# vbarbosadev/MatrixFactorizationSGD.java

Hardware: AMD Instinct MI355X
Metric: rating-updates/sec (higher is better)
Workload: dtype f32; 1 GPU; cfg2_ml20m (MovieLens-20M shape, Zipf-Mandelbrot degrees); workload_rev=2, users_per_gpu=138493, items=26744, nnz_per_gpu=20000000, nnz_global=20000000, users_global=138493, k=64, max_item_degree=67853, sum_round_steps=51381, blocks=256, waves=2, parts_per_rank=1, emulated_world=0, parallelism=single

## Files before the change

### matrixfactorizationsgd.java_amd/csrc/cell.hpp

```cpp
#pragma once

#include <hip/hip_runtime.h>

#include <cstdint>

#include "canon.hpp"
#include "records.hpp"
#include "run_asm.hpp"

#pragma clang fp contract(off)

namespace mfsgd {
namespace {

__device__ __forceinline__ void wg_barrier() { asm volatile("s_waitcnt lgkmcnt(0)\n\ts_barrier" ::: "memory"); }

using gptr_t = const __attribute__((address_space(1))) void*;
using lptr_t = __attribute__((address_space(3))) void*;
using f32x4 = __attribute__((ext_vector_type(4))) float;

__device__ __forceinline__ float4 lds_ld(const unsigned char* base, unsigned off) {
    return *reinterpret_cast<const float4*>(base + off);
}
__device__ __forceinline__ void lds_st(unsigned char* base, unsigned off, const float4 v) {
    *reinterpret_cast<float4*>(base + off) = v;
}

template <int EST, int L>
__device__ __forceinline__ void run_loop_asm(float4& rq, const unsigned ea, const unsigned rowbase, int pairs,
                                             const float lr) {
    static_assert(L == 16 || L == 32 || L == 64, "hand-scheduled run loop: 16, 32 or 64 lanes per rating");
    using f4 = __attribute__((ext_vector_type(4))) float;
    f4 q = {rq.x, rq.y, rq.z, rq.w};
    constexpr int PADV = mfsgd_pad_run(L);
    if constexpr (L == 16)
        asm volatile(MFSGD_RUN_LOOP_ASM_TEXT("", MFSGD_SFMA_V) MFSGD_RUN_LOOP_ASM_OPERANDS);
    else if constexpr (L == 32)
        asm volatile(MFSGD_RUN_LOOP_ASM_TEXT(MFSGD_SWAP_ADD16, MFSGD_SFMA_V) MFSGD_RUN_LOOP_ASM_OPERANDS);
    else
        asm volatile(MFSGD_RUN_LOOP_ASM_TEXT(MFSGD_BCAST_ADD64, MFSGD_SFMA_S) MFSGD_RUN_LOOP_ASM_OPERANDS);
    rq = make_float4(q[0], q[1], q[2], q[3]);
}

template <int EST, int L>
__device__ __forceinline__ void gen_loop_asm(const unsigned ea, const unsigned rowbase, int n, const float lr, const uint64_t c2) {
    static_assert(L == 16 || L == 32 || L == 64, "hand-scheduled general loop: 16, 32 or 64 lanes per rating");
    n = __builtin_amdgcn_readfirstlane(n);
    constexpr int PADV = mfsgd_pad_gen(L);
    if constexpr (L == 16)
        asm volatile(MFSGD_GEN_LOOP_ASM_TEXT("", MFSGD_SFMA_V) MFSGD_GEN_LOOP_ASM_OPERANDS);
    else if constexpr (L == 32)
        asm volatile(MFSGD_GEN_LOOP_ASM_TEXT(MFSGD_SWAP_ADD16, MFSGD_SFMA_V) MFSGD_GEN_LOOP_ASM_OPERANDS);
    else
        asm volatile(MFSGD_GEN_LOOP_ASM_TEXT(MFSGD_BCAST_ADD64, MFSGD_SFMA_S) MFSGD_GEN_LOOP_ASM_OPERANDS);
}

template <int L>
__device__ __forceinline__ void solo_chain_asm(float4& rq, const unsigned ea, const unsigned s0, const unsigned rowbase, int n,
                                               const float lr, const uint64_t c2) {
    static_assert(L == 16 || L == 32 || L == 64, "solo loops: 16, 32 or 64 lanes per rating");
    using f4 = __attribute__((ext_vector_type(4))) float;
    f4 q;
    n = __builtin_amdgcn_readfirstlane(n);
    constexpr int PADV = mfsgd_pad_chain_tail(L), PADS = mfsgd_pad_chain_steady(L);
    if constexpr (L == 16)
        asm volatile(MFSGD_SOLO_CHAIN_ASM_TEXT("", MFSGD_SFMA2_V) MFSGD_SOLO_CHAIN_OPERANDS);
    else if constexpr (L == 32)
        asm volatile(MFSGD_SOLO_CHAIN_ASM_TEXT(MFSGD_BCAST_ADD32, MFSGD_SFMA2_S) MFSGD_SOLO_CHAIN_OPERANDS);
    else
        asm volatile(MFSGD_SOLO_CHAIN_ASM_TEXT(MFSGD_BCAST_ADD64, MFSGD_SFMA2_S) MFSGD_SOLO_CHAIN_OPERANDS);
    rq = make_float4(q[0], q[1], q[2], q[3]);
}
template <int L>
__device__ __forceinline__ bool solo_helper_asm(const unsigned ea, const unsigned rowbase, int n, const uint64_t c2,
                                                int fin = 1) {
    constexpr int PADV = mfsgd_pad_helper(L);
    n = __builtin_amdgcn_readfirstlane(n);
    fin = __builtin_amdgcn_readfirstlane(fin);
    asm volatile("" : "+s"(fin));
    int spins = 1 << 22;
    asm volatile(MFSGD_SOLO_HELPER_ASM_TEXT MFSGD_SOLO_HELPER_OPERANDS);
    return spins != 0;
}

template <int L, int W>
constexpr int epoch_helpers() {
    return W <= 4 ? W : 0;
}

__device__ __forceinline__ CellDesc load_desc(const CellDesc* __restrict__ cells, unsigned idx) {
    idx = (unsigned)__builtin_amdgcn_readfirstlane((int)idx);
    asm volatile("" : "+s"(idx));
    return cells[idx];
}

template <int L, int W, int NH = 0>
struct Cell {
    static constexpr int G = 64 / L;
    static constexpr int ROWB = 16 * L;
    static constexpr int KP = 4 * L;
    static constexpr int NWV = W + NH;
    static constexpr int NT = 64 * NWV;
    static constexpr int CTL = 16;
    static constexpr int SUBB = (W * W * 8 + 15) & ~15;

    int tid, lane, wave, g, lig;
    int wave_all;
    bool helper;
    unsigned laneoff;
    int nu, nrows, n_steps;
    bool critical;
    volatile unsigned* fail_flag = nullptr;
    unsigned long long* post_at = nullptr;
    unsigned post_tag = 0;
    volatile unsigned* posted_flag = nullptr;
    unsigned char* lrows;
    uint4* lent;
    uint2* lsub;
    uint32_t* lids;

    __device__ __forceinline__ void init_thread() {
        tid = threadIdx.x;
        lane = tid & 63;
        wave_all = __builtin_amdgcn_readfirstlane(tid >> 6);
        helper = NH > 0 && wave_all >= W;
        wave = helper ? wave_all - W : wave_all;
        g = lane / L;
        lig = lane % L;
        laneoff = (unsigned)lig * 16u;
    }
    __device__ __forceinline__ void bind(const CellDesc& cd, unsigned char* smem, int buf, int sched_cap) {
        nu = cd.nu;
        nrows = (int)cd.nu + (int)cd.ni;
        n_steps = (int)(cd.n_steps & 0x7FFFFFFFu);
        critical = (cd.n_steps >> 31) != 0;
        lrows = smem + CTL + 2 * (size_t)sched_cap;
        lent = reinterpret_cast<uint4*>(smem + CTL + (size_t)buf * sched_cap);
        lsub = reinterpret_cast<uint2*>(lent + (size_t)n_steps * G);
        lids = reinterpret_cast<uint32_t*>(reinterpret_cast<unsigned char*>(lsub) + SUBB);
    }

    __device__ __forceinline__ void zero_idle_rows() {
        for (int x = tid; x < 2 * G * L; x += NT)
            lds_st(lrows, (unsigned)(nrows * ROWB + x * 16), make_float4(0.f, 0.f, 0.f, 0.f));
    }

    __device__ __forceinline__ void prefetch_schedule(const CellDesc& nd, int ncell, unsigned char* smem, int buf,
                                                      int sched_cap, const uint32_t* __restrict__ rows,
                                                      const SubDesc* __restrict__ subs,
                                                      const Entry* __restrict__ entries) {
        unsigned char* const dst = smem + CTL + (size_t)buf * sched_cap;
        const int nn = (int)nd.nu + (int)nd.ni;
        const int ent_bytes = (int)(nd.n_steps & 0x7FFFFFFFu) * G * 16;
        const int sub_bytes = SUBB;
        const int ids_bytes = (nn * 4 + 15) & ~15;
        auto copy = [&](const unsigned char* src, unsigned char* d, int bytes) {
            for (int off0 = wave_all * 1024; off0 < bytes; off0 += NWV * 1024) {
                const int off = off0 + lane * 16;
                if (off < bytes)
                    __builtin_amdgcn_global_load_lds((gptr_t)(src + off), (lptr_t)(d + off0), 16, 0, 0);
            }
        };
        copy(reinterpret_cast<const unsigned char*>(entries + (size_t)nd.ent_off * G), dst, ent_bytes);
        copy(reinterpret_cast<const unsigned char*>(subs + (size_t)ncell * W * W), dst + ent_bytes, sub_bytes);
        copy(reinterpret_cast<const unsigned char*>(rows + nd.row_off), dst + ent_bytes + sub_bytes, ids_bytes);
    }

    __device__ __forceinline__ void stage_schedule(const CellDesc& cd, int cell, const uint32_t* __restrict__ rows,
                                                   const SubDesc* __restrict__ subs,
                                                   const Entry* __restrict__ entries) {
        const uint32_t* const crow = rows + cd.row_off;
        for (int x = tid; x < nrows; x += NT) lids[x] = crow[x];
        const uint4* gent = reinterpret_cast<const uint4*>(entries) + (size_t)cd.ent_off * G;
        const int ne = n_steps * G;
        for (int x = tid; x < ne; x += NT) lent[x] = gent[x];
        if (tid < W * W) lsub[tid] = reinterpret_cast<const uint2*>(subs)[(size_t)cell * W * W + tid];
        zero_idle_rows();
    }

    template <bool COH = false>
    __device__ __forceinline__ void gather(const float* __restrict__ P, const float* __restrict__ Q, int lo, int hi) {
        constexpr int AUX = COH ? 16 : 0;
        constexpr int UNR = 4;
        const int first = (lo / G) * G;
        int s0 = first + wave_all * G;
        for (; s0 + (UNR - 1) * NWV * G < hi; s0 += UNR * NWV * G) {
            uint32_t rid[UNR];
            bool in[UNR];
#pragma unroll
            for (int x = 0; x < UNR; ++x) {
                const int sx = s0 + x * NWV * G + g;
                in[x] = sx >= lo && sx < hi;
                rid[x] = lids[in[x] ? sx : lo];
            }
#pragma unroll
            for (int x = 0; x < UNR; ++x) {
                const int sb = s0 + x * NWV * G;
                if (in[x]) {
                    const float* src = (sb + g < nu ? P : Q) + (size_t)rid[x] * KP + lig * 4;
                    __builtin_amdgcn_global_load_lds((gptr_t)src, (lptr_t)(lrows + (size_t)sb * ROWB), 16, 0, AUX);
                }
            }
        }
        for (; s0 < hi; s0 += NWV * G) {
            const int sx = s0 + g;
            if (sx >= lo && sx < hi) {
                const uint32_t rid = lids[sx];
                const float* src = (sx < nu ? P : Q) + (size_t)rid * KP + lig * 4;
                __builtin_amdgcn_global_load_lds((gptr_t)src, (lptr_t)(lrows + (size_t)s0 * ROWB), 16, 0, AUX);
            }
        }
    }

    template <bool WT>
    __device__ __forceinline__ void scatter(float* __restrict__ P, float* __restrict__ Q, int lo, int hi) {
        constexpr int UNR = 4;
        auto put = [&](int s, uint32_t rid, const float4 v) {
            float* dst = (s < nu ? P : Q) + (size_t)rid * KP + lig * 4;
            if constexpr (WT) {
                const f32x4 vv = {v.x, v.y, v.z, v.w};
                asm volatile("s_nop 1\n\tglobal_store_dwordx4 %0, %1, off sc1\n\ts_nop 1" ::"v"(dst), "v"(vv) : "memory");
            } else {
                *reinterpret_cast<float4*>(dst) = v;
            }
        };
        int s = lo + wave_all * G + g;
        for (; s + (UNR - 1) * NWV * G < hi; s += UNR * NWV * G) {
            uint32_t rid[UNR];
            float4 v[UNR];
#pragma unroll
            for (int x = 0; x < UNR; ++x) {
                rid[x] = lids[s + x * NWV * G];
                v[x] = lds_ld(lrows, (unsigned)((s + x * NWV * G) * ROWB) + laneoff);
            }
#pragma unroll
            for (int x = 0; x < UNR; ++x) put(s + x * NWV * G, rid[x], v[x]);
        }
        for (; s < hi; s += NWV * G) put(s, lids[s], lds_ld(lrows, (unsigned)(s * ROWB) + laneoff));
    }

    struct Sub {
        int n, nr;
        int offs;
        __device__ __forceinline__ int first() const { return offs & 0xFFFF; }
        __device__ __forceinline__ int nsolo() const { return (int)((unsigned)offs >> 16); }
    };
    __device__ __forceinline__ Sub sub(const int x) const {
        const uint2 sd = lsub[x];
        const int nall = __builtin_amdgcn_readfirstlane((int)sd.y);
        return Sub{nall & 0xFFFF, (int)((unsigned)nall >> 16), __builtin_amdgcn_readfirstlane((int)sd.x)};
    }
    static __device__ __forceinline__ uint64_t pack_c2(const float c) {
        return ((uint64_t)__builtin_bit_cast(unsigned, c) << 32) | __builtin_bit_cast(unsigned, c);
    }
    static __device__ __forceinline__ unsigned row_base(unsigned char* rows, const unsigned lo) {
        return (unsigned)(uintptr_t)(lptr_t)rows + lo;
    }
    static constexpr bool kAsmLoops = L == 16 || L == 32 || L == 64;

    struct StepRegs {
        uint4 en;
        unsigned pa, qa;
        float4 p, q;
    };

    template <bool TRAIN, bool TIMED = false>
    __device__ __forceinline__ void apply(const float lr, const float c, double& acc,
                                          unsigned long long* timers = nullptr) {
        unsigned char* const lr_ = lrows;
        const unsigned lo = laneoff;
        if constexpr (NH > 0 && TRAIN) {
            if (helper) {
                for (int s = 0; s < W; ++s) {
                    if constexpr (L >= 16) {
                        auto run_of = [&](const int a, int& ns) -> const uint4* {
                            const uint2 sd = lsub[s * W + a];
                            ns = __builtin_amdgcn_readfirstlane((int)(sd.x >> 16));
                            const int first = __builtin_amdgcn_readfirstlane((int)((sd.x & 0xFFFFu) + (sd.y & 0xFFFFu) + (sd.y >> 16))) + kSoloPad;
                            return lent + (size_t)first * G;
                        };
                        int ns;
                        const uint4* hdr = run_of((wave + 1) % W, ns);
                        if (ns > 0 && !solo_helper_asm<L>((unsigned)(uintptr_t)(lptr_t)hdr, row_base(lr_, lo), ns, pack_c2(c)) && fail_flag)
                            *fail_flag = 1;
                    }
                    wg_barrier();
                }
                return;
            }
        }
        auto set_addr = [&](StepRegs& x) {
            x.pa = ((x.en.x & 0xFFFFu) << 4) + lo;
            x.qa = (__builtin_amdgcn_ubfe(x.en.x, 16, 15) << 4) + lo;
        };
        auto step = [&](StepRegs& cur, StepRegs& nxt, const uint4* eptr, const int e2) {
            __builtin_amdgcn_sched_barrier(0);
            asm volatile("" : "+v"(nxt.en.x));
            const float r = __builtin_bit_cast(float, TRAIN ? cur.en.z : cur.en.y);
            set_addr(nxt);
            const float4 pn = lds_ld(lr_, nxt.pa);
            const float4 qn = lds_ld(lr_, nxt.qa);
            cur.en = eptr[e2];
            __builtin_amdgcn_sched_barrier(0);
            const float dot = group_allreduce<L>(chunk_dot(cur.p, cur.q));
            if constexpr (TRAIN) {
                const float sc = __builtin_fmaf(-lr, dot, r);
                const float4 p2 = axpy_row(sc, cur.q, c, cur.p);
                const float4 q2 = axpy_row(sc, cur.p, c, cur.q);
                lds_st(lr_, cur.pa, p2);
                lds_st(lr_, cur.qa, q2);
                const bool fwd = (int)nxt.en.x < 0;
                nxt.q.x = fwd ? q2.x : qn.x;
                nxt.q.y = fwd ? q2.y : qn.y;
                nxt.q.z = fwd ? q2.z : qn.z;
                nxt.q.w = fwd ? q2.w : qn.w;
            } else {
                const float err = r - dot;
                acc += (double)err * (double)err;
                nxt.q = qn;
            }
            nxt.p = pn;
// ... 145 lines not shown
```

### matrixfactorizationsgd.java_amd/csrc/epoch.hip

```cpp
#include <hip/hip_runtime.h>

#include <cstdint>

#include "cell.hpp"
#include "dispatch.hpp"
#include "kernels.hpp"

#pragma clang fp contract(off)

namespace mfsgd {

namespace {

constexpr int kFlagStride = 32;

using gu32 = __attribute__((address_space(1))) unsigned;
using gu64 = __attribute__((address_space(1))) unsigned long long;

__device__ __forceinline__ unsigned start_barrier(unsigned* __restrict__ done, unsigned* __restrict__ abort_word,
                                                  const int B, const int wg, const int NP, unsigned& my_gen) {
    unsigned bad = __hip_atomic_load((gu32*)abort_word, __ATOMIC_RELAXED, __HIP_MEMORY_SCOPE_AGENT);
    my_gen = 0;
    if (bad == 0u) {
        gu32* arrive = (gu32*)(abort_word - 4);
// ... 65 lines not shown
__device__ __forceinline__ void post_row(gu64* dst, const unsigned long long tag, const int lane,
                                         const unsigned char* row) {
#pragma unroll
    for (int j = 0; j < NGR; ++j) {
        const unsigned bits = *reinterpret_cast<const unsigned*>(row + (size_t)(lane + 64 * j) * 4);
        __hip_atomic_store(dst + 64 * j, tag | bits, __ATOMIC_RELAXED, __HIP_MEMORY_SCOPE_AGENT);
    }
}

template <int L, int W, int NH>
__device__ __forceinline__ void run_ring(unsigned char* smem, float* __restrict__ P, float* __restrict__ Q,
                                         const CellDesc* __restrict__ cells, const uint32_t* __restrict__ rows,
                                         const SubDesc* __restrict__ subs, const Entry* __restrict__ entries,
                                         const int B, const int n_rounds, const float lr, const float c,
                                         unsigned* __restrict__ done, unsigned* __restrict__ abort_word,
                                         const int sched_cap, const int wg, const int NP,
                                         unsigned long long* __restrict__ prof) {
    volatile unsigned* const ctl = reinterpret_cast<volatile unsigned*>(smem);
    Cell<L, W, NH> cx;
    cx.init_thread();
    cx.fail_flag = ctl;
    cx.posted_flag = ctl + 3;
    if (cx.tid == 0) {
        unsigned my_gen;
        const unsigned bad = start_barrier(done, abort_word, B, wg, NP, my_gen);
        ctl[0] = bad != 0u ? 1u : 0u;
        ctl[1] = bad;
        ctl[2] = my_gen;
    }
    wg_barrier();
    if (ctl[0] != 0) return;
    gu64* const mbox = (gu64*)(abort_word + 4);
    const unsigned tag_hi = ctl[2] << 16;
    constexpr int KP = Cell<L, W, NH>::KP, ROWB = Cell<L, W, NH>::ROWB;
    constexpr int NGR = KP >= 64 ? KP / 64 : 1;

    struct Item {
        int R, b;
        unsigned idx;
        bool first;
    };
    auto cell_of = [&](int R, int b) { return (unsigned)(b * B + (b + R % B) % B); };
    auto next_item = [&](const Item& it, const CellDesc& d) {
        Item n = it;
        if (d.next != 0) {
            n.idx = d.next;
            n.first = false;
        } else {
            n.b += NP;
            if (n.b >= B) {
                n.b = wg;
                ++n.R;
            }
            n.idx = cell_of(n.R, n.b);
            n.first = true;
        }
        return n;
    };
    Item it0{0, wg, cell_of(0, wg), true};
    CellDesc cd = load_desc(cells, it0.idx);
    Item it1 = next_item(it0, cd);
    CellDesc cd1 = it1.R < n_rounds ? load_desc(cells, it1.idx) : cd;
    int buf = 0;
    cx.bind(cd, smem, buf, sched_cap);
    cx.stage_schedule(cd, (int)it0.idx, rows, subs, entries);
    asm volatile("s_waitcnt vmcnt(0)" ::: "memory");
    wg_barrier();

    unsigned long long pacc[8] = {0, 0, 0, 0, 0, 0, 0, 0};
    unsigned long long pcur[7] = {0, 0, 0, 0, 0, 0, 0}, pmax[7] = {0, 0, 0, 0, 0, 0, 0};
    unsigned long long pt = 0;
    auto mark = [&](int k) {
        if (prof) {
            const unsigned long long now = __builtin_amdgcn_s_memtime();
            pacc[k] += now - pt;
            pcur[k] = now - pt;
            if (k == 6 && pcur[4] > pacc[7]) {
                pacc[7] = pcur[4];
                for (int x = 0; x < 7; ++x) pmax[x] = pcur[x];
            }
            pt = now;
        }
    };
    if (prof) pt = __builtin_amdgcn_s_memtime();

    for (; it0.R < n_rounds;) {
        const int R = it0.R, b = it0.b;
        CellDesc cd2 = cd1;
        cx.bind(cd, smem, buf, sched_cap);
        const bool work = cx.nrows != 0;
        const bool last = cd.next == 0;
        cx.zero_idle_rows();
        if (cx.tid == 0) ctl[3] = 0u;
        asm volatile("s_waitcnt vmcnt(0)" ::: "memory");
#ifdef MFSGD_DIAG_SPLIT_PHASE0
        mark(0);
#endif
        if (it1.R < n_rounds) cx.prefetch_schedule(cd1, (int)it1.idx, smem, buf ^ 1, sched_cap, rows, subs, entries);
        if (work) cx.gather(P, Q, 0, cx.nu);
        const Item it2 = next_item(it1, cd1);
        const bool lone = KP >= 64 && (cd.rsv[0] & kCellLoneTile) != 0;
#ifdef MFSGD_DIAG_SPLIT_PHASE0
        mark(2);
#endif
        if (it2.R < n_rounds) cd2 = load_desc(cells, it2.idx);
#ifdef MFSGD_DIAG_SPLIT_PHASE0
        mark(6);
#else
        mark(0);
#endif
        if (R > 0 && it0.first && lone) {
            if (cx.wave_all == 0) {
                const unsigned tile = (unsigned)((b + R % B) % B);
                const unsigned want = tag_hi | (unsigned)R;
                const gu64* src = mbox + (size_t)tile * KP + cx.lane;
                unsigned long long v[NGR];
                unsigned spins = 0;
                for (;;) {
                    bool ok = true;
#pragma unroll
                    for (int j = 0; j < NGR; ++j) {
                        v[j] = __hip_atomic_load(src + 64 * j, __ATOMIC_RELAXED, __HIP_MEMORY_SCOPE_AGENT);
                        ok = ok && (unsigned)(v[j] >> 32) == want;
                    }
                    if (__builtin_amdgcn_ballot_w64(!ok) == 0ull) break;
                    __builtin_amdgcn_s_sleep(1);
                    if ((++spins & 255u) == 0u) {
                        if (__hip_atomic_load((gu32*)abort_word, __ATOMIC_RELAXED, __HIP_MEMORY_SCOPE_AGENT) != 0u ||
                            spins > (1u << 22)) {
                            if (cx.lane == 0) {
                                __hip_atomic_store((gu32*)abort_word, 1u, __ATOMIC_RELAXED, __HIP_MEMORY_SCOPE_AGENT);
                                ctl[0] = 1;
                            }
                            break;
                        }
                    }
                }
#pragma unroll
                for (int j = 0; j < NGR; ++j)
                    *reinterpret_cast<unsigned*>(cx.lrows + (size_t)cx.nu * ROWB + (size_t)(cx.lane + 64 * j) * 4) = (unsigned)v[j];
            }
        } else if (R > 0 && it0.first) {
            if (cx.tid == 0) {
                wait_flag((gu32*)(done + (size_t)((b + 1) % B) * kFlagStride), (unsigned)R, abort_word, ctl);
            }
        }
        mark(1);
        const bool from_mbox = lone && R > 0;
        wg_barrier();
        mark(2);
        if (ctl[0] != 0) {
            if (cx.tid == 0) __hip_atomic_store((gu32*)abort_word, 1u, __ATOMIC_RELAXED, __HIP_MEMORY_SCOPE_AGENT);
            return;
        }
        if (work && !from_mbox) cx.template gather<true>(P, Q, cx.nu, cx.nrows);
        if (work) {
            asm volatile("s_waitcnt vmcnt(0)" ::: "memory");
            wg_barrier();
            mark(3);
            double acc = 0.0;
            if (lone && R + 1 < n_rounds) {
                cx.post_at = (unsigned long long*)(abort_word + 4) + (size_t)((b + R % B) % B) * KP;
                cx.post_tag = tag_hi | (unsigned)(R + 1);
            } else {
                cx.post_at = nullptr;
            }
            cx.template apply<true>(lr, c, acc);
            mark(4);
            if (lone && R + 1 < n_rounds) {
                if (cx.wave_all == 0 && ctl[3] == 0u) {
                    const unsigned tile = (unsigned)((b + R % B) % B);
                    const unsigned long long tag = (unsigned long long)(tag_hi | (unsigned)(R + 1)) << 32;
                    post_row<NGR>(mbox + (size_t)tile * KP + cx.lane, tag, cx.lane, cx.lrows + (size_t)cx.nu * ROWB);
                }
            } else {
                cx.template scatter<true>(P, Q, cx.nu, cx.nrows);
            }
        }
        asm volatile("s_waitcnt vmcnt(0)" ::: "memory");
        wg_barrier();
        if (last && cx.tid == 0)
            __hip_atomic_store((gu32*)(done + (size_t)b * kFlagStride), (unsigned)(R + 1), __ATOMIC_RELAXED,
                               __HIP_MEMORY_SCOPE_AGENT);
        mark(5);
        if (work) cx.template scatter<false>(P, Q, 0, cx.nu);
        wg_barrier();
        buf ^= 1;
        cd = cd1;
        cd1 = cd2;
        it0 = it1;
        it1 = it2;
        mark(6);
    }
    if (ctl[0] != 0 && cx.tid == 0)
        __hip_atomic_store((gu32*)abort_word, 1u, __ATOMIC_RELAXED, __HIP_MEMORY_SCOPE_AGENT);
    if (wg == 0 && cx.tid == 0)
        __hip_atomic_fetch_add((gu32*)(abort_word + 1), 1u, __ATOMIC_RELAXED, __HIP_MEMORY_SCOPE_AGENT);
    if (prof && cx.tid == 0) {
        for (int k = 0; k < 8; ++k) prof[(size_t)wg * 16 + k] = pacc[k];
        for (int k = 0; k < 7; ++k) prof[(size_t)wg * 16 + 8 + k] = pmax[k];
    }
}

template <int L, int W>
__global__ void __launch_bounds__(64 * (W + epoch_helpers<L, W>()))
epoch_kernel(float* __restrict__ P, float* __restrict__ Q, const CellDesc* __restrict__ cells,
             const uint32_t* __restrict__ rows, const SubDesc* __restrict__ subs,
             const Entry* __restrict__ entries, const int B, const int n_rounds, const float lr,
             const float c, unsigned* __restrict__ done, unsigned* __restrict__ abort_word,
             const int sched_cap, unsigned long long* __restrict__ prof) {
    extern __shared__ __attribute__((aligned(16))) unsigned char smem[];
    run_ring<L, W, epoch_helpers<L, W>()>(smem, P, Q, cells, rows, subs, entries, B, n_rounds, lr, c, done, abort_word,
                                           sched_cap, (int)blockIdx.x, (int)gridDim.x, prof);
}

template <int L, int W>
hipError_t epoch_grant_lds(const CellLaunch& a) {
    return hipFuncSetAttribute((const void*)epoch_kernel<L, W>, hipFuncAttributeMaxDynamicSharedMemorySize, a.lds_bytes);
}

template <int L, int W>
hipError_t epoch_occupancy_LW(const CellLaunch& a, int* blocks_per_cu) {
    const hipError_t e = epoch_grant_lds<L, W>(a);
    if (e != hipSuccess) return e;
    return hipOccupancyMaxActiveBlocksPerMultiprocessor(blocks_per_cu, (const void*)epoch_kernel<L, W>,
                                                        64 * (W + epoch_helpers<L, W>()), (size_t)a.lds_bytes);
}

template <int L, int W>
hipError_t epoch_launch_LW(const CellLaunch& a, int n_rounds, unsigned* done, unsigned* abort_word, hipStream_t st) {
    const hipError_t e = epoch_grant_lds<L, W>(a);
    if (e != hipSuccess) return e;
    hipLaunchKernelGGL((epoch_kernel<L, W>), dim3((unsigned)a.grid), dim3(64 * (W + epoch_helpers<L, W>())),
                       (size_t)a.lds_bytes, st, a.P, a.Q, a.cells, a.rows, a.subs, a.entries, a.B, n_rounds, a.lr, a.c, done,
                       abort_word, a.sched_cap, reinterpret_cast<unsigned long long*>(a.diag ? a.sse_partial : nullptr));
    return hipGetLastError();
}

}

hipError_t epoch_blocks_per_cu(int L, int W, const CellLaunch& a, int* blocks_per_cu) {
    return with_L(L, [&](auto l) { return with_W(W, [&](auto w) { return epoch_occupancy_LW<l(), w()>(a, blocks_per_cu); }); });
}

hipError_t launch_epoch_persistent(int L, int W, const CellLaunch& a, int n_rounds, unsigned* done,
                                   unsigned* abort_word, hipStream_t st) {
    return with_L(L, [&](auto l) {
        return with_W(W, [&](auto w) { return epoch_launch_LW<l(), w()>(a, n_rounds, done, abort_word, st); });
    });
}

}
```

### matrixfactorizationsgd.java_amd/csrc/run_asm.hpp

```cpp
#pragma once

constexpr int mfsgd_pad_run(int lanes) {
#ifdef MFSGD_PAD_RUN
    return MFSGD_PAD_RUN;
#else
    return 2;
#endif
}
constexpr int mfsgd_pad_gen(int lanes) {
#ifdef MFSGD_PAD_GEN
    return MFSGD_PAD_GEN;
#else
    return 0;
#endif
}
constexpr int mfsgd_pad_chain_steady(int lanes) {
#ifdef MFSGD_PAD_CHAIN_STEADY
    return MFSGD_PAD_CHAIN_STEADY;
#else
    return 0;
#endif
}
constexpr int mfsgd_pad_chain_tail(int lanes) {
#ifdef MFSGD_PAD_CHAIN_TAIL
// ... 144 lines not shown
        EXTRA \
        SFMA(LRR) \
        "v_pk_fma_f32 v[" NQ0 ":" NQ1 "], v[130:131], v[" P0 ":" P1 "], v[122:123] op_sel_hi:[0,1,1]\n\t" \
        "v_pk_fma_f32 v[" NQ2 ":" NQ3 "], v[130:131], v[" P2 ":" P3 "], v[124:125] op_sel_hi:[0,1,1]\n\t" \
        "v_pk_fma_f32 v[134:135], v[130:131], v[" Q0 ":" Q1 "], v[126:127] op_sel_hi:[0,1,1]\n\t" \
        "v_pk_fma_f32 v[136:137], v[130:131], v[" Q2 ":" Q3 "], v[128:129] op_sel_hi:[0,1,1]\n\t" \
        "s_sub_u32 %[n], %[n], 1\n\t" \
        "v_cmp_gt_i32 vcc, 0, v" SLOT_NEXT "\n\t" \
        "ds_write_b128 v" PADDR ", v[134:137]\n\t" \
        "ds_write_b128 v" QADDR ", v[" NQ0 ":" NQ3 "]\n\t" \
        "s_cmp_eq_u32 %[n], 0\n\t" \
        "s_waitcnt lgkmcnt(4)\n\t" \
        "v_cndmask_b32 v" NQ0 ", v144, v" NQ0 ", vcc\n\t" \
        "v_cndmask_b32 v" NQ1 ", v145, v" NQ1 ", vcc\n\t" \
        "v_cndmask_b32 v" NQ2 ", v146, v" NQ2 ", vcc\n\t" \
        "v_cndmask_b32 v" NQ3 ", v147, v" NQ3 ", vcc\n\t"

#define MFSGD_GEN_LOOP_ASM_TEXT(EXTRA, SFMA) \
        "v_mov_b32 v138, %[ea]\n\t" \
        "v_mov_b32 v131, %[lr]\n\t" \
        "v_mov_b32 v139, %[rb]\n\t" \
        "ds_read_b32 v114, v138\n\t" \
        "ds_read_b32 v116, v138 offset:8\n\t" \
        "ds_read_b32 v115, v138 offset:%c[e1]\n\t" \
        "s_waitcnt lgkmcnt(2)\n\t" \
        "v_mad_u32_u16 v112, v114, 16, v139\n\t" \
        "v_bfe_u32 v133, v114, 16, 15\n\t" \
        "v_lshl_add_u32 v148, v133, 4, v139\n\t" \
        "ds_read_b128 v[104:107], v112\n\t" \
        "ds_read_b128 v[100:103], v148\n\t" \
        "ds_write_b32 v138, v114\n\t" \
        "ds_write_b32 v138, v114\n\t" \
        MFSGD_LOOP_ALIGN \
        "1:\n\t" \
        MFSGD_GEN_HALF("104", "105", "106", "107", "100", "101", "102", "103", "112", "148", "108", "111", "140", "141", "142", "143", \
                       "113", "149", "115", "114", "%c[e2]", "116", "117", "%c[e1p8]", EXTRA, SFMA) \
        "s_cbranch_scc1 2f\n\t" \
        MFSGD_GEN_HALF("108", "109", "110", "111", "140", "141", "142", "143", "113", "149", "104", "107", "100", "101", "102", "103", \
                       "112", "148", "114", "115", "%c[e3]", "117", "116", "%c[e2p8]", EXTRA, SFMA) \
        "v_add_u32 v138, %c[e2], v138\n\t" \
        "s_cbranch_scc0 1b\n\t" \
        "2:\n\t" \
        "s_waitcnt lgkmcnt(0)\n\t"

#define MFSGD_GEN_LOOP_ASM_OPERANDS                                                                                    \
    : [n] "+s"(n)                                                                                                      \
    : [ea] "v"(ea), [rb] "v"(rowbase), [lr] "s"(lr), [c2] "s"(c2), [e1] "n"(EST), [e2] "n"(2 * EST), [e3] "n"(3 * EST), \
      [e1p8] "n"(EST + 8), [e2p8] "n"(2 * EST + 8), [pad] "n"(PADV)                                                    \
    : "memory", "scc", "vcc", "v100", "v101", "v102", "v103", "v104", "v105", "v106", "v107", "v108", "v109", "v110", "v111", \
      "v112", "v113", "v114", "v115", "v116", "v117", "v120", "v121", "v122", "v123", "v124", "v125", "v126", "v127",  \
      "v128", "v129", "v130", "v131", "v132", "v133", "v134", "v135", "v136", "v137", "v138", "v139", "v140", "v141",  \
      "v142", "v143", "v144", "v145", "v146", "v147", "v148", "v149"

#define MFSGD_SOLO_CHAIN_HALF(P0, P1, P2, P3, N0, N1, N2, N3, ELRR, ESLOT, NEXTE, OFF_NEXT, WAIT, S, S1, GAP, EXTRA, SFMA) \
        "s_waitcnt lgkmcnt(" WAIT ")\n\t" \
        "v_pk_mul_f32 v[120:121], v[" P0 ":" P1 "], v[100:101]\n\t" \
        "v_pk_fma_f32 v[120:121], v[" P2 ":" P3 "], v[102:103], v[120:121]\n\t" \
        "v_add_f32 v132, v120, v121\n\t" \
        "v_mad_u32_u16 v113, v" ESLOT ", 16, v139\n\t" \
        "v_pk_mul_f32 v[122:123], v[100:101], %[c2]\n\t" \
        "v_add_f32_dpp v132, v132, v132 quad_perm:[1,0,3,2] row_mask:0xf bank_mask:0xf bound_ctrl:1\n\t" \
        "ds_read_b128 v[" N0 ":" N3 "], v113\n\t" \
        "v_pk_mul_f32 v[124:125], v[102:103], %[c2]\n\t" \
        "v_add_f32_dpp v132, v132, v132 quad_perm:[2,3,0,1] row_mask:0xf bank_mask:0xf bound_ctrl:1\n\t" \
        "ds_read2_b32 v[" NEXTE "], v138 " OFF_NEXT "\n\t" \
        "s_nop 0\n\t" \
        "v_add_f32_dpp v132, v132, v132 row_half_mirror row_mask:0xf bank_mask:0xf bound_ctrl:1\n\t" \
        GAP \
        "v_add_f32_dpp v132, v132, v132 row_mirror row_mask:0xf bank_mask:0xf bound_ctrl:1\n\t" \
        EXTRA \
        SFMA(S, ELRR) \
        "v_pk_fma_f32 v[100:101], v[" S ":" S1 "], v[" P0 ":" P1 "], v[122:123] op_sel_hi:[0,1,1]\n\t" \
        "v_pk_fma_f32 v[102:103], v[" S ":" S1 "], v[" P2 ":" P3 "], v[124:125] op_sel_hi:[0,1,1]\n\t"

#define MFSGD_SOLO_CHAIN_GAP_COUNT "s_sub_u32 %[n], %[n], 1\n\ts_cmp_eq_u32 %[n], 0\n\t"
#define MFSGD_SOLO_CHAIN_GAP_NOP "s_nop 1\n\t"
#define MFSGD_SOLO_CHAIN_GAP_PASS \
        ".if 2 * \\j + 2 < %c[steady]\n\ts_nop 1\n\t.else\n\ts_sub_u32 %[n], %[n], %c[steady]\n\ts_cmp_ge_u32 %[n], %c[steady]\n\t.endif\n\t"
#define MFSGD_SOLO_CHAIN_PAIR(GAP_A, GAP_B, EXIT_A, EXTRA, SFMA) \
        MFSGD_SOLO_CHAIN_HALF("104", "105", "106", "107", "108", "109", "110", "111", "116", "117", "118:119", "offset0:6+8*\\j offset1:4+8*\\j", "1", "130", "131", GAP_A, EXTRA, SFMA) \
        EXIT_A \
        MFSGD_SOLO_CHAIN_HALF("108", "109", "110", "111", "104", "105", "106", "107", "118", "119", "116:117", "offset0:10+8*\\j offset1:8+8*\\j", "0", "128", "129", GAP_B, EXTRA, SFMA) \
        "ds_write2_b32 v138, v130, v128 offset0:1+8*\\j offset1:5+8*\\j\n\t"
#define MFSGD_SOLO_CHAIN_ASM_TEXT(EXTRA, SFMA) \
        "v_mov_b32 v138, %[ea]\n\t" \
        "v_mov_b32 v131, %[lr]\n\t" \
        "v_mov_b32 v139, %[rb]\n\t" \
        "ds_read2_b32 v[116:117], v138 offset0:6 offset1:4\n\t" \
        "v_mad_u32_u16 v113, %[s0], 16, v139\n\t" \
        "v_bfe_u32 v133, %[s0], 16, 15\n\t" \
        "ds_read_b128 v[104:107], v113\n\t" \
        "v_lshl_add_u32 v133, v133, 4, v139\n\t" \
        "ds_read_b128 v[100:103], v133\n\t" \
        "ds_write_b32 v138, %[s0]\n\t" \
        "v_add_u32 v138, 16, v138\n\t" \
        "s_cmp_lt_u32 %[n], %c[steady]\n\t" \
        "s_cbranch_scc1 1f\n\t" \
        MFSGD_LOOP_ALIGN_STEADY \
        "5:\n\t" \
        ".irp j,0,1,2,3,4,5,6,7\n\t" \
        ".if 2 * \\j < %c[steady]\n\t" \
        MFSGD_SOLO_CHAIN_PAIR(MFSGD_SOLO_CHAIN_GAP_NOP, MFSGD_SOLO_CHAIN_GAP_PASS, "", EXTRA, SFMA) \
        ".endif\n\t" \
        ".endr\n\t" \
        "v_add_u32 v138, %c[sbump], v138\n\t" \
        "s_cbranch_scc1 5b\n\t" \
        "s_cmp_eq_u32 %[n], 0\n\t" \
        "s_cbranch_scc1 3f\n\t" \
        "s_branch 1f\n\t" \
        MFSGD_LOOP_ALIGN \
        "1:\n\t" \
        ".irp j,0,1,2,3\n\t" \
        ".if \\j < %c[pairs]\n\t" \
        MFSGD_SOLO_CHAIN_PAIR(MFSGD_SOLO_CHAIN_GAP_COUNT, MFSGD_SOLO_CHAIN_GAP_COUNT, "s_cbranch_scc1 2\\j\\()f\n\t", EXTRA, SFMA) \
        ".if \\j + 1 < %c[pairs]\n\t" \
        "s_cbranch_scc1 3f\n\t" \
        ".endif\n\t" \
        ".endif\n\t" \
        ".endr\n\t" \
        "v_add_u32 v138, %c[bump], v138\n\t" \
        "s_cbranch_scc0 1b\n\t" \
        "s_branch 3f\n\t" \
        ".irp j,3,2,1,0\n\t" \
        ".if \\j < %c[pairs]\n\t" \
        "2\\j:\n\t" \
        "ds_write_b32 v138, v130 offset:4+32*\\j\n\t" \
        ".if \\j > 0\n\t" \
        "s_branch 3f\n\t" \
        ".endif\n\t" \
        ".endif\n\t" \
        ".endr\n\t" \
        "3:\n\t" \
        "s_waitcnt lgkmcnt(0)\n\t" \
        "v_mov_b32 %[q0], v100\n\t" \
        "v_mov_b32 %[q1], v101\n\t" \
        "v_mov_b32 %[q2], v102\n\t" \
        "v_mov_b32 %[q3], v103\n\t"

#define MFSGD_SOLO_CHAIN_OPERANDS                                                                                      \
    : [n] "+s"(n), [q0] "=v"(q[0]), [q1] "=v"(q[1]), [q2] "=v"(q[2]), [q3] "=v"(q[3])                                  \
    : [ea] "v"(ea), [rb] "v"(rowbase), [s0] "v"(s0), [lr] "s"(lr), [c2] "s"(c2), [pad] "n"(PADV),                      \
      [pads] "n"(PADS), [pairs] "n"(mfsgd_chain_pairs()), [bump] "n"(32 * mfsgd_chain_pairs()),                         \
      [steady] "n"(mfsgd_chain_steady()), [sbump] "n"(16 * mfsgd_chain_steady())                                       \
    : "memory", "scc", "vcc", "v100", "v101", "v102", "v103", "v104", "v105", "v106", "v107", "v108", "v109", "v110", "v111", \
      "v113", "v116", "v117", "v118", "v119", "v120", "v121", "v122", "v123", "v124", "v125", "v128", "v129", "v130",  \
      "v131", "v132", "v133", "v138", "v139"

#define MFSGD_SOLO_HELPER_PAIR(TAG, M0, M1, M2, M3, N0, N3) \
        "s_waitcnt lgkmcnt(1)\n\t" \
        "v_max_u32 v133, v" M1 ", v" M3 "\n\t" \
        "v_mad_u32_u16 v113, v" M0 ", 16, v139\n\t" \
        "v_cmp_eq_u32 vcc, -1, v133\n\t" \
        "v_pk_mul_f32 v[126:127], v[104:105], %[c2]\n\t" \
        "s_cbranch_vccnz 7" TAG "f\n\t" \
        "6" TAG ":\n\t" \
        "ds_read_b128 v[108:111], v113\n\t" \
        "v_pk_mul_f32 v[128:129], v[106:107], %[c2]\n\t" \
        "ds_read2_b64 v[" N0 ":" N3 "], v138 offset0:4 offset1:6\n\t" \
        "v_pk_mul_f32 v[122:123], v[100:101], %[c2]\n\t" \
        "v_pk_mul_f32 v[124:125], v[102:103], %[c2]\n\t" \
        "v_pk_fma_f32 v[134:135], v[" M0 ":" M1 "], v[100:101], v[126:127] op_sel:[1,0,0]\n\t" \
        "v_pk_fma_f32 v[136:137], v[" M0 ":" M1 "], v[102:103], v[128:129] op_sel:[1,0,0]\n\t" \
        "v_pk_fma_f32 v[100:101], v[" M0 ":" M1 "], v[104:105], v[122:123] op_sel:[1,0,0]\n\t" \
        "v_pk_fma_f32 v[102:103], v[" M0 ":" M1 "], v[106:107], v[124:125] op_sel:[1,0,0]\n\t" \
        "s_sub_u32 %[n], %[n], 2\n\t" \
        "ds_write_b128 v112, v[134:137]\n\t" \
        "v_mad_u32_u16 v112, v" M2 ", 16, v139\n\t" \
        "s_waitcnt lgkmcnt(2)\n\t" \
        "ds_read_b128 v[104:107], v112\n\t" \
        "v_pk_mul_f32 v[126:127], v[108:109], %[c2]\n\t" \
        "v_pk_mul_f32 v[128:129], v[110:111], %[c2]\n\t" \
        "v_pk_mul_f32 v[122:123], v[100:101], %[c2]\n\t" \
        "v_pk_mul_f32 v[124:125], v[102:103], %[c2]\n\t" \
        "v_pk_fma_f32 v[134:135], v[" M2 ":" M3 "], v[100:101], v[126:127] op_sel:[1,0,0]\n\t" \
        "v_pk_fma_f32 v[136:137], v[" M2 ":" M3 "], v[102:103], v[128:129] op_sel:[1,0,0]\n\t" \
        "v_pk_fma_f32 v[100:101], v[" M2 ":" M3 "], v[108:109], v[122:123] op_sel:[1,0,0]\n\t" \
        "v_pk_fma_f32 v[102:103], v[" M2 ":" M3 "], v[110:111], v[124:125] op_sel:[1,0,0]\n\t" \
        "v_add_u32 v138, 32, v138\n\t" \
        "s_cmp_lt_u32 %[n], 2\n\t" \
        "ds_write_b128 v113, v[134:137]\n\t"

#define MFSGD_SOLO_HELPER_SLOW(TAG, M0, M1, M3) \
        "7" TAG ":\n\t" \
        "s_sleep 1\n\t" \
        "ds_read2_b64 v[" M0 ":" M3 "], v138 offset1:2\n\t" \
        "s_sub_u32 %[spins], %[spins], 1\n\t" \
        "s_cmp_eq_u32 %[spins], 0\n\t" \
        "s_cbranch_scc1 9f\n\t" \
        "s_waitcnt lgkmcnt(0)\n\t" \
        "v_max_u32 v133, v" M1 ", v" M3 "\n\t" \
        "v_cmp_eq_u32 vcc, -1, v133\n\t" \
        "s_cbranch_vccnz 7" TAG "b\n\t" \
        "s_branch 6" TAG "b\n\t"

#define MFSGD_SOLO_HELPER_TAIL(TAG, M0, M1) \
        "8" TAG ":\n\t" \
        "s_cmp_eq_u32 %[n], 0\n\t" \
        "s_cbranch_scc1 40f\n\t" \
        "s_waitcnt lgkmcnt(0)\n\t" \
        "v_pk_mul_f32 v[126:127], v[104:105], %[c2]\n\t" \
        "v_pk_mul_f32 v[128:129], v[106:107], %[c2]\n\t" \
        "v_pk_mul_f32 v[122:123], v[100:101], %[c2]\n\t" \
        "v_pk_mul_f32 v[124:125], v[102:103], %[c2]\n\t" \
        "3" TAG ":\n\t" \
        "v_cmp_eq_u32 vcc, -1, v" M1 "\n\t" \
        "s_cbranch_vccz 2" TAG "f\n\t" \
        "s_sleep 1\n\t" \
        "ds_read_b32 v" M1 ", v138 offset:4\n\t" \
        "s_sub_u32 %[spins], %[spins], 1\n\t" \
        "s_cmp_eq_u32 %[spins], 0\n\t" \
        "s_cbranch_scc1 9f\n\t" \
        "s_waitcnt lgkmcnt(0)\n\t" \
        "s_branch 3" TAG "b\n\t" \
        "2" TAG ":\n\t" \
        "v_pk_fma_f32 v[134:135], v[" M0 ":" M1 "], v[100:101], v[126:127] op_sel:[1,0,0]\n\t" \
        "v_pk_fma_f32 v[136:137], v[" M0 ":" M1 "], v[102:103], v[128:129] op_sel:[1,0,0]\n\t" \
        "v_pk_fma_f32 v[100:101], v[" M0 ":" M1 "], v[104:105], v[122:123] op_sel:[1,0,0]\n\t" \
        "v_pk_fma_f32 v[102:103], v[" M0 ":" M1 "], v[106:107], v[124:125] op_sel:[1,0,0]\n\t" \
        "s_nop 0\n\t" \
        "ds_write_b128 v112, v[134:137]\n\t"

#define MFSGD_SOLO_HELPER_ASM_TEXT \
        "v_mov_b32 v141, %[ea]\n\t" \
        "v_mov_b32 v139, %[rb]\n\t" \
        "ds_read_b32 v133, v141\n\t" \
        "v_add_u32 v138, 16, v141\n\t" \
        "3:\n\t" \
        "ds_read2_b64 v[116:119], v138 offset1:2\n\t" \
        "s_waitcnt lgkmcnt(0)\n\t" \
// ... 42 lines not shown
```

Before: 5.441 billion updates/s.

## Fuse lone-tile mailbox poll, solo chain and row post into one asm loop

Adds a fast path for lone tiles whose round contains only a solo chain. One inline-asm block now polls the mailbox for the incoming row, runs the solo SGD chain on it and posts the updated row to the next tile's mailbox. This removes the separate poll loop, the barriers, the gather/apply dispatch and the post_row pass on the critical inter-block handoff chain. The cost is much more hand-written asm, extra clobbered VGPRs, and narrower eligibility checks that fall back to the old path.

```diff
diff --git a/matrixfactorizationsgd.java_amd/csrc/cell.hpp b/matrixfactorizationsgd.java_amd/csrc/cell.hpp
--- a/matrixfactorizationsgd.java_amd/csrc/cell.hpp
+++ b/matrixfactorizationsgd.java_amd/csrc/cell.hpp
@@ -83,6 +83,31 @@
     return spins != 0;
 }
 
+template <int L>
+__device__ __forceinline__ bool lone_chain_asm(const unsigned ea, const unsigned s0, const unsigned rowbase, int n, const float lr,
+                                               const uint64_t c2, const __attribute__((address_space(1))) unsigned long long* src,
+                                               unsigned want, const __attribute__((address_space(1))) unsigned* abw,
+                                               const unsigned ctl, __attribute__((address_space(1))) unsigned long long* dst,
+                                               unsigned ptag, uint64_t pm, unsigned prof) {
+    static_assert(L == 16 || L == 32 || L == 64, "solo loops: 16, 32 or 64 lanes per rating");
+    n = __builtin_amdgcn_readfirstlane(n);
+    pm = (uint64_t)(unsigned)__builtin_amdgcn_readfirstlane((int)(unsigned)pm) |
+         (uint64_t)(unsigned)__builtin_amdgcn_readfirstlane((int)(unsigned)(pm >> 32)) << 32;
+    want = (unsigned)__builtin_amdgcn_readfirstlane((int)want);
+    ptag = (unsigned)__builtin_amdgcn_readfirstlane((int)ptag);
+    prof = (unsigned)__builtin_amdgcn_readfirstlane((int)prof);
+    unsigned spins = 0, gave = 0, t0;
+    uint64_t tmp;
+    constexpr int PADV = mfsgd_pad_chain_tail(L), PADS = mfsgd_pad_chain_steady(L);
+    if constexpr (L == 16)
+        asm volatile(MFSGD_LONE_CHAIN_ASM_TEXT("", MFSGD_SFMA2_V) MFSGD_LONE_CHAIN_OPERANDS);
+    else if constexpr (L == 32)
+        asm volatile(MFSGD_LONE_CHAIN_ASM_TEXT(MFSGD_BCAST_ADD32, MFSGD_SFMA2_S) MFSGD_LONE_CHAIN_OPERANDS);
+    else
+        asm volatile(MFSGD_LONE_CHAIN_ASM_TEXT(MFSGD_BCAST_ADD64, MFSGD_SFMA2_S) MFSGD_LONE_CHAIN_OPERANDS);
+    return gave == 0;
+}
+
 template <int L, int W>
 constexpr int epoch_helpers() {
     return W <= 4 ? W : 0;
@@ -237,6 +262,50 @@
             for (int x = 0; x < UNR; ++x) put(s + x * NWV * G, rid[x], v[x]);
         }
         for (; s < hi; s += NWV * G) put(s, lids[s], lds_ld(lrows, (unsigned)(s * ROWB) + laneoff));
+    }
+
+    __device__ __forceinline__ bool lone_solo_only() const {
+        if constexpr (NH > 0 && kAsmLoops && W * W <= 64) {
+            const uint2 sd = lsub[lane < W * W ? lane : 0];
+            const int nsolo = (int)(sd.x >> 16);
+            const bool ok = lane == 0 ? (sd.x & 0xFFFFu) == 0u && sd.y == 0u && nsolo > 0 &&
+                                            (nsolo + 2 + G - 1) / G + kSoloPad + 2 == n_steps
+                                      : lane >= W * W || (sd.y == 0u && nsolo == 0);
+            return __builtin_amdgcn_ballot_w64(!ok) == 0ull;
+        } else {
+            return false;
+        }
+    }
+    __device__ __forceinline__ bool lone_round0(const float lr, const float c,
+                                                const __attribute__((address_space(1))) unsigned long long* src,
+                                                const unsigned want, const __attribute__((address_space(1))) unsigned* abw,
+                                                volatile unsigned* ctl, const bool prof) {
+        const uint4* const hdr = lent + (size_t)kSoloPad * G;
+        if constexpr (NH > 0 && kAsmLoops) {
+            if (wave_all == 0) {
+                const unsigned s0 = hdr->x;
+                const int nsolo = __builtin_amdgcn_readfirstlane((int)(lsub[0].x >> 16));
+                const bool post = post_at != nullptr;
+                const uint64_t pm = !post ? 0ull : L == 64 ? ~0ull : (1ull << (L & 63)) - 1ull;
+                auto* dst = (__attribute__((address_space(1))) unsigned long long*)post_at + lig * 4;
+                const bool ok = lone_chain_asm<L>((unsigned)(uintptr_t)(lptr_t)hdr, s0, row_base(lrows, laneoff), nsolo, lr, pack_c2(c),
+                                                  src + lig * 4, want, abw, (unsigned)(uintptr_t)(lptr_t)ctl, dst, post_tag, pm,
+                                                  prof ? 1u : 0u);
+                if (!ok) return false;
+                if (post && lane == 0) *posted_flag = 1u;
+                for (int s = 0; s < W; ++s) wg_barrier();
+                return true;
+            }
+            int ns = 0;
+            const bool mine = helper && (wave + 1) % W == 0;
+            if (mine) ns = __builtin_amdgcn_readfirstlane((int)(lsub[0].x >> 16));
+            wg_barrier();
+            if (ctl[0] != 0) return false;
+            if (mine && !solo_helper_asm<L>((unsigned)(uintptr_t)(lptr_t)hdr, row_base(lrows, laneoff), ns, pack_c2(c)) && fail_flag)
+                *fail_flag = 1;
+            for (int s = 0; s < W; ++s) wg_barrier();
+        }
+        return true;
     }
 
     struct Sub {
diff --git a/matrixfactorizationsgd.java_amd/csrc/epoch.hip b/matrixfactorizationsgd.java_amd/csrc/epoch.hip
--- a/matrixfactorizationsgd.java_amd/csrc/epoch.hip
+++ b/matrixfactorizationsgd.java_amd/csrc/epoch.hip
@@ -171,6 +171,12 @@
             pt = now;
         }
     };
+    auto mark_at = [&](int k, const unsigned now_lo) {
+        const unsigned long long now = pt + (unsigned long long)(now_lo - (unsigned)pt);
+        pacc[k] += now - pt;
+        pcur[k] = now - pt;
+        pt = now;
+    };
     if (prof) pt = __builtin_amdgcn_s_memtime();
 
     for (; it0.R < n_rounds;) {
@@ -198,72 +204,99 @@
 #else
         mark(0);
 #endif
-        if (R > 0 && it0.first && lone) {
-            if (cx.wave_all == 0) {
-                const unsigned tile = (unsigned)((b + R % B) % B);
-                const unsigned want = tag_hi | (unsigned)R;
-                const gu64* src = mbox + (size_t)tile * KP + cx.lane;
-                unsigned long long v[NGR];
-                unsigned spins = 0;
-                for (;;) {
-                    bool ok = true;
-#pragma unroll
-                    for (int j = 0; j < NGR; ++j) {
-                        v[j] = __hip_atomic_load(src + 64 * j, __ATOMIC_RELAXED, __HIP_MEMORY_SCOPE_AGENT);
-                        ok = ok && (unsigned)(v[j] >> 32) == want;
-                    }
-                    if (__builtin_amdgcn_ballot_w64(!ok) == 0ull) break;
-                    __builtin_amdgcn_s_sleep(1);
-                    if ((++spins & 255u) == 0u) {
-                        if (__hip_atomic_load((gu32*)abort_word, __ATOMIC_RELAXED, __HIP_MEMORY_SCOPE_AGENT) != 0u ||
-                            spins > (1u << 22)) {
-                            if (cx.lane == 0) {
-                                __hip_atomic_store((gu32*)abort_word, 1u, __ATOMIC_RELAXED, __HIP_MEMORY_SCOPE_AGENT);
-                                ctl[0] = 1;
-                            }
-                            break;
-                        }
-                    }
-                }
-#pragma unroll
-                for (int j = 0; j < NGR; ++j)
-                    *reinterpret_cast<unsigned*>(cx.lrows + (size_t)cx.nu * ROWB + (size_t)(cx.lane + 64 * j) * 4) = (unsigned)v[j];
-            }
-        } else if (R > 0 && it0.first) {
-            if (cx.tid == 0) {
-                wait_flag((gu32*)(done + (size_t)((b + 1) % B) * kFlagStride), (unsigned)R, abort_word, ctl);
-            }
-        }
-        mark(1);
-        const bool from_mbox = lone && R > 0;
-        wg_barrier();
-        mark(2);
-        if (ctl[0] != 0) {
-            if (cx.tid == 0) __hip_atomic_store((gu32*)abort_word, 1u, __ATOMIC_RELAXED, __HIP_MEMORY_SCOPE_AGENT);
-            return;
-        }
-        if (work && !from_mbox) cx.template gather<true>(P, Q, cx.nu, cx.nrows);
-        if (work) {
+        const bool fast = R > 0 && it0.first && lone && cx.lone_solo_only();
+        if (fast) {
             asm volatile("s_waitcnt vmcnt(0)" ::: "memory");
             wg_barrier();
-            mark(3);
-            double acc = 0.0;
-            if (lone && R + 1 < n_rounds) {
-                cx.post_at = (unsigned long long*)(abort_word + 4) + (size_t)((b + R % B) % B) * KP;
+            mark(2);
+            if (ctl[0] != 0) {
+                if (cx.tid == 0) __hip_atomic_store((gu32*)abort_word, 1u, __ATOMIC_RELAXED, __HIP_MEMORY_SCOPE_AGENT);
+                return;
+            }
+            const unsigned tile = (unsigned)((b + R % B) % B);
+            if (R + 1 < n_rounds) {
+                cx.post_at = (unsigned long long*)(mbox + (size_t)tile * KP);
                 cx.post_tag = tag_hi | (unsigned)(R + 1);
             } else {
                 cx.post_at = nullptr;
             }
-            cx.template apply<true>(lr, c, acc);
+            if (!cx.lone_round0(lr, c, mbox + (size_t)tile * KP, tag_hi | (unsigned)R, (gu32*)abort_word, ctl, prof != nullptr))
+                return;
+            if (prof) {
+                const unsigned arrived = ctl[1];
+                mark_at(1, arrived);
+                mark_at(3, arrived);
+            }
             mark(4);
-            if (lone && R + 1 < n_rounds) {
-                if (cx.wave_all == 0 && ctl[3] == 0u) {
+            if (R + 1 >= n_rounds) cx.template scatter<true>(P, Q, cx.nu, cx.nrows);
+        } else {
+            if (R > 0 && it0.first && lone) {
+                if (cx.wave_all == 0) {
                     const unsigned tile = (unsigned)((b + R % B) % B);
-                    const unsigned long long tag = (unsigned long long)(tag_hi | (unsigned)(R + 1)) << 32;
-                    post_row<NGR>(mbox + (size_t)tile * KP + cx.lane, tag, cx.lane, cx.lrows + (size_t)cx.nu * ROWB);
-                }
-            } else {
-                cx.template scatter<true>(P, Q, cx.nu, cx.nrows);
+                    const unsigned want = tag_hi | (unsigned)R;
+                    const gu64* src = mbox + (size_t)tile * KP + cx.lane;
+                    unsigned long long v[NGR];
+                    unsigned spins = 0;
+                    for (;;) {
+                        bool ok = true;
+#pragma unroll
+                        for (int j = 0; j < NGR; ++j) {
+                            v[j] = __hip_atomic_load(src + 64 * j, __ATOMIC_RELAXED, __HIP_MEMORY_SCOPE_AGENT);
+                            ok = ok && (unsigned)(v[j] >> 32) == want;
+                        }
+                        if (__builtin_amdgcn_ballot_w64(!ok) == 0ull) break;
+                        __builtin_amdgcn_s_sleep(1);
+                        if ((++spins & 255u) == 0u) {
+                            if (__hip_atomic_load((gu32*)abort_word, __ATOMIC_RELAXED, __HIP_MEMORY_SCOPE_AGENT) != 0u ||
+                                spins > (1u << 22)) {
+                                if (cx.lane == 0) {
+                                    __hip_atomic_store((gu32*)abort_word, 1u, __ATOMIC_RELAXED, __HIP_MEMORY_SCOPE_AGENT);
+                                    ctl[0] = 1;
+                                }
+                                break;
+                            }
+                        }
+                    }
+#pragma unroll
+                    for (int j = 0; j < NGR; ++j)
+                        *reinterpret_cast<unsigned*>(cx.lrows + (size_t)cx.nu * ROWB + (size_t)(cx.lane + 64 * j) * 4) = (unsigned)v[j];
+                }
+            } else if (R > 0 && it0.first) {
+                if (cx.tid == 0) {
+                    wait_flag((gu32*)(done + (size_t)((b + 1) % B) * kFlagStride), (unsigned)R, abort_word, ctl);
+                }
+            }
+            mark(1);
+            const bool from_mbox = lone && R > 0;
+            wg_barrier();
+            mark(2);
+            if (ctl[0] != 0) {
+                if (cx.tid == 0) __hip_atomic_store((gu32*)abort_word, 1u, __ATOMIC_RELAXED, __HIP_MEMORY_SCOPE_AGENT);
+                return;
+            }
+            if (work && !from_mbox) cx.template gather<true>(P, Q, cx.nu, cx.nrows);
+            if (work) {
+                asm volatile("s_waitcnt vmcnt(0)" ::: "memory");
+                wg_barrier();
+                mark(3);
+                double acc = 0.0;
+                if (lone && R + 1 < n_rounds) {
+                    cx.post_at = (unsigned long long*)(abort_word + 4) + (size_t)((b + R % B) % B) * KP;
+                    cx.post_tag = tag_hi | (unsigned)(R + 1);
+                } else {
+                    cx.post_at = nullptr;
+                }
+                cx.template apply<true>(lr, c, acc);
+                mark(4);
+                if (lone && R + 1 < n_rounds) {
+                    if (cx.wave_all == 0 && ctl[3] == 0u) {
+                        const unsigned tile = (unsigned)((b + R % B) % B);
+                        const unsigned long long tag = (unsigned long long)(tag_hi | (unsigned)(R + 1)) << 32;
+                        post_row<NGR>(mbox + (size_t)tile * KP + cx.lane, tag, cx.lane, cx.lrows + (size_t)cx.nu * ROWB);
+                    }
+                } else {
+                    cx.template scatter<true>(P, Q, cx.nu, cx.nrows);
+                }
             }
         }
         asm volatile("s_waitcnt vmcnt(0)" ::: "memory");
diff --git a/matrixfactorizationsgd.java_amd/csrc/run_asm.hpp b/matrixfactorizationsgd.java_amd/csrc/run_asm.hpp
--- a/matrixfactorizationsgd.java_amd/csrc/run_asm.hpp
+++ b/matrixfactorizationsgd.java_amd/csrc/run_asm.hpp
@@ -250,19 +250,7 @@
         EXIT_A \
         MFSGD_SOLO_CHAIN_HALF("108", "109", "110", "111", "104", "105", "106", "107", "118", "119", "116:117", "offset0:10+8*\\j offset1:8+8*\\j", "0", "128", "129", GAP_B, EXTRA, SFMA) \
         "ds_write2_b32 v138, v130, v128 offset0:1+8*\\j offset1:5+8*\\j\n\t"
-#define MFSGD_SOLO_CHAIN_ASM_TEXT(EXTRA, SFMA) \
-        "v_mov_b32 v138, %[ea]\n\t" \
-        "v_mov_b32 v131, %[lr]\n\t" \
-        "v_mov_b32 v139, %[rb]\n\t" \
-        "ds_read2_b32 v[116:117], v138 offset0:6 offset1:4\n\t" \
-        "v_mad_u32_u16 v113, %[s0], 16, v139\n\t" \
-        "v_bfe_u32 v133, %[s0], 16, 15\n\t" \
-        "ds_read_b128 v[104:107], v113\n\t" \
-        "v_lshl_add_u32 v133, v133, 4, v139\n\t" \
-        "ds_read_b128 v[100:103], v133\n\t" \
-        "ds_write_b32 v138, %[s0]\n\t" \
-        "v_add_u32 v138, 16, v138\n\t" \
-        "s_cmp_lt_u32 %[n], %c[steady]\n\t" \
+#define MFSGD_SOLO_CHAIN_BODIES(EXTRA, SFMA) \
         "s_cbranch_scc1 1f\n\t" \
         MFSGD_LOOP_ALIGN_STEADY \
         "5:\n\t" \
@@ -297,7 +285,22 @@
         "s_branch 3f\n\t" \
         ".endif\n\t" \
         ".endif\n\t" \
-        ".endr\n\t" \
+        ".endr\n\t"
+
+#define MFSGD_SOLO_CHAIN_ASM_TEXT(EXTRA, SFMA) \
+        "v_mov_b32 v138, %[ea]\n\t" \
+        "v_mov_b32 v131, %[lr]\n\t" \
+        "v_mov_b32 v139, %[rb]\n\t" \
+        "ds_read2_b32 v[116:117], v138 offset0:6 offset1:4\n\t" \
+        "v_mad_u32_u16 v113, %[s0], 16, v139\n\t" \
+        "v_bfe_u32 v133, %[s0], 16, 15\n\t" \
+        "ds_read_b128 v[104:107], v113\n\t" \
+        "v_lshl_add_u32 v133, v133, 4, v139\n\t" \
+        "ds_read_b128 v[100:103], v133\n\t" \
+        "ds_write_b32 v138, %[s0]\n\t" \
+        "v_add_u32 v138, 16, v138\n\t" \
+        "s_cmp_lt_u32 %[n], %c[steady]\n\t" \
+        MFSGD_SOLO_CHAIN_BODIES(EXTRA, SFMA) \
         "3:\n\t" \
         "s_waitcnt lgkmcnt(0)\n\t" \
         "v_mov_b32 %[q0], v100\n\t" \
@@ -313,6 +316,103 @@
     : "memory", "scc", "vcc", "v100", "v101", "v102", "v103", "v104", "v105", "v106", "v107", "v108", "v109", "v110", "v111", \
       "v113", "v116", "v117", "v118", "v119", "v120", "v121", "v122", "v123", "v124", "v125", "v128", "v129", "v130",  \
       "v131", "v132", "v133", "v138", "v139"
+
+#ifdef MFSGD_LONE_POLL_NO_SLEEP
+#define MFSGD_LONE_POLL_SLEEP ""
+#else
+#define MFSGD_LONE_POLL_SLEEP "s_sleep 1\n\t"
+#endif
+#define MFSGD_LONE_CHAIN_ASM_TEXT(EXTRA, SFMA) \
+        "v_mov_b32 v138, %[ea]\n\t" \
+        "v_mov_b32 v131, %[lr]\n\t" \
+        "v_mov_b32 v139, %[rb]\n\t" \
+        "ds_read2_b32 v[116:117], v138 offset0:6 offset1:4\n\t" \
+        "v_mad_u32_u16 v113, %[s0], 16, v139\n\t" \
+        "v_bfe_u32 v133, %[s0], 16, 15\n\t" \
+        "ds_read_b128 v[104:107], v113\n\t" \
+        "v_lshl_add_u32 v133, v133, 4, v139\n\t" \
+        "v_add_u32 v138, 16, v138\n\t" \
+        "v_mov_b32 v151, %[ptag]\n\t" \
+        "v_mov_b32 v153, %[ptag]\n\t" \
+        "v_mov_b32 v155, %[ptag]\n\t" \
+        "v_mov_b32 v157, %[ptag]\n\t" \
+        "v_mov_b32 v149, 0\n\t" \
+        "s_waitcnt lgkmcnt(0)\n\t" \
+        "60:\n\t" \
+        "global_load_dwordx2 v[100:101], %[src], off sc1\n\t" \
+        "global_load_dwordx2 v[142:143], %[src], off offset:8 sc1\n\t" \
+        "global_load_dwordx2 v[144:145], %[src], off offset:16 sc1\n\t" \
+        "global_load_dwordx2 v[146:147], %[src], off offset:24 sc1\n\t" \
+        "s_waitcnt vmcnt(0)\n\t" \
+        "v_xor_b32 v101, %[want], v101\n\t" \
+        "v_xor_b32 v143, %[want], v143\n\t" \
+        "v_xor_b32 v145, %[want], v145\n\t" \
+        "v_xor_b32 v147, %[want], v147\n\t" \
+        "v_or3_b32 v101, v101, v143, v145\n\t" \
+        "v_or_b32 v101, v101, v147\n\t" \
+        "v_cmp_ne_u32 vcc, 0, v101\n\t" \
+        "s_cbranch_vccz 62f\n\t" \
+        MFSGD_LONE_POLL_SLEEP \
+        "s_add_u32 %[spins], %[spins], 1\n\t" \
+        "s_and_b32 %[t0], %[spins], 0xff\n\t" \
+        "s_cbranch_scc1 60b\n\t" \
+        "global_load_dword v148, v149, %[abw] sc1\n\t" \
+        "s_waitcnt vmcnt(0)\n\t" \
+        "v_readfirstlane_b32 %[t0], v148\n\t" \
+        "s_cmp_lg_u32 %[t0], 0\n\t" \
+        "s_cbranch_scc1 61f\n\t" \
+        "s_cmp_le_u32 %[spins], 0x400000\n\t" \
+        "s_cbranch_scc1 60b\n\t" \
+        "61:\n\t" \
+        "v_mov_b32 v148, 1\n\t" \
+        "s_mov_b64 %[tmp], exec\n\t" \
+        "s_mov_b64 exec, 1\n\t" \
+        "global_store_dword v149, v148, %[abw] sc1\n\t" \
+        "ds_write_b32 %[ctl], v148\n\t" \
+        "s_mov_b64 exec, %[tmp]\n\t" \
+        "s_mov_b32 %[gave], 1\n\t" \
+        "s_waitcnt vmcnt(0) lgkmcnt(0)\n\t" \
+        "s_barrier\n\t" \
+        "s_branch 69f\n\t" \
+        "62:\n\t" \
+        "v_mov_b32 v101, v142\n\t" \
+        "v_mov_b32 v102, v144\n\t" \
+        "v_mov_b32 v103, v146\n\t" \
+        "s_cmp_eq_u32 %[prof], 0\n\t" \
+        "s_cbranch_scc1 63f\n\t" \
+        "s_memtime %[tmp]\n\t" \
+        "s_waitcnt lgkmcnt(0)\n\t" \
+        "v_mov_b64 v[158:159], %[tmp]\n\t" \
+        "ds_write_b32 %[ctl], v158 offset:4\n\t" \
+        "63:\n\t" \
+        "s_cmp_lt_u32 %[n], %c[steady]\n\t" \
+        "ds_write_b128 v133, v[100:103]\n\t" \
+        "s_barrier\n\t" \
+        MFSGD_SOLO_CHAIN_BODIES(EXTRA, SFMA) \
+        "3:\n\t" \
+        "v_mov_b32 v150, v100\n\t" \
+        "v_mov_b32 v152, v101\n\t" \
+        "v_mov_b32 v154, v102\n\t" \
+        "v_mov_b32 v156, v103\n\t" \
+        "s_and_saveexec_b64 %[tmp], %[pm]\n\t" \
+        "global_store_dwordx2 %[dst], v[150:151], off sc1\n\t" \
+        "global_store_dwordx2 %[dst], v[152:153], off offset:8 sc1\n\t" \
+        "global_store_dwordx2 %[dst], v[154:155], off offset:16 sc1\n\t" \
+        "global_store_dwordx2 %[dst], v[156:157], off offset:24 sc1\n\t" \
+        "s_mov_b64 exec, %[tmp]\n\t" \
+        "69:\n\t" \
+        "s_waitcnt lgkmcnt(0)\n\t"
+
+#define MFSGD_LONE_CHAIN_OPERANDS                                                                                      \
+    : [n] "+s"(n), [spins] "+s"(spins), [gave] "+s"(gave), [tmp] "=&s"(tmp), [t0] "=&s"(t0)                            \
+    : [ea] "v"(ea), [rb] "v"(rowbase), [s0] "v"(s0), [lr] "s"(lr), [c2] "s"(c2), [src] "v"(src), [want] "s"(want),     \
+      [abw] "s"(abw), [ctl] "v"(ctl), [dst] "v"(dst), [ptag] "s"(ptag), [pm] "s"(pm), [prof] "s"(prof),                \
+      [pad] "n"(PADV), [pads] "n"(PADS), [pairs] "n"(mfsgd_chain_pairs()), [bump] "n"(32 * mfsgd_chain_pairs()),        \
+      [steady] "n"(mfsgd_chain_steady()), [sbump] "n"(16 * mfsgd_chain_steady())                                       \
+    : "memory", "scc", "vcc", "v100", "v101", "v102", "v103", "v104", "v105", "v106", "v107", "v108", "v109", "v110", "v111", \
+      "v113", "v116", "v117", "v118", "v119", "v120", "v121", "v122", "v123", "v124", "v125", "v128", "v129", "v130",  \
+      "v131", "v132", "v133", "v138", "v139", "v142", "v143", "v144", "v145", "v146", "v147", "v148", "v149", "v150",  \
+      "v151", "v152", "v153", "v154", "v155", "v156", "v157", "v158", "v159"
 
 #define MFSGD_SOLO_HELPER_PAIR(TAG, M0, M1, M2, M3, N0, N3) \
         "s_waitcnt lgkmcnt(1)\n\t" \
```

Measured after the change: 5.606 billion updates/s (median of 6 runs). 3.0% higher.
